# OedonLestrange42/GNURadio-WiFI-ImageTransfer

Measured on NVIDIA B200. Metric: rx_msamples_per_s, higher is better.
Workload: dtype f32+u8

## Files before the change

### gnuradio-wifi-imagetransfer_b200/csrc/rx_kernels.cuh

```cuda
#pragma once
#include <cuda_pipeline.h>
#include "viterbi.cuh"

__device__ __forceinline__ cf fe_at(const cf *x, int64_t j, int hist) { return j < -(int64_t)hist ? cf{0.f, 0.f} : x[j]; }

__device__ __forceinline__ int find_link(const LinkDesc *links, int n_links, int64_t chunk)
{
    int lo = 0, hi = n_links - 1;
    while (lo < hi) {
        int mid = (lo + hi + 1) >> 1;
        if (links[mid].chunk_base <= chunk) lo = mid; else hi = mid - 1;
    }
    return lo;
}

#ifndef DET_BLOCK
#define DET_BLOCK 32
#endif
#define DET_SPLIT (DET_THREADS / DET_BLOCK)
#define DET_ROWS (DET_BLOCK + 2)
#define DET_STRIDE 66
#define DET_SMEM_BYTES (DET_ROWS * DET_STRIDE * (int)sizeof(cf) + 32)

__device__ __forceinline__ uint32_t det_smem_u32(const void *p) { return (uint32_t)__cvta_generic_to_shared(p); }
// ... 775 lines not shown
                        if (k == 32 || k < 6 || k > 58) continue;
                        sum = cadd(sum, s_hu[wib][k]);
                        ++cnt;
                    }
                    cf avg = {sum.re / (float)cnt, sum.im / (float)cnt};
                    if (u) HB = cadd(cscale(HB, 0.5f), cscale(avg, 0.5f));
                    else HA = cadd(cscale(HA, 0.5f), cscale(avg, 0.5f));
                }
                __syncwarp();
            }
            if (PHASE == 0) {
                if (carA >= 0) st->sig_bits[carA] = (uint8_t)bitsA;
                if (carB >= 0) st->sig_bits[carB] = (uint8_t)bitsB;
            } else {
                int64_t row = F.row_off + (n - 3);
                if (carA >= 0) rows[row * 48 + carA] = (uint8_t)bitsA;
                if (carB >= 0) rows[row * 48 + carB] = (uint8_t)bitsB;
                if (prm.want_carrier) {
                    if (carA >= 0) carrier[row * 48 + carA] = symA;
                    if (carB >= 0) carrier[row * 48 + carB] = symB;
                }
                if (wps) {
                    if (carA >= 0)
                        *reinterpret_cast<uint2 *>(&s_bits[wib][carA * 8]) =
                            make_uint2((((uint32_t)bitsA & 15u) * 0x00204081u) & 0x01010101u, (((uint32_t)bitsA >> 4) * 0x81u) & 0x0101u);
                    if (carB >= 0)
                        *reinterpret_cast<uint2 *>(&s_bits[wib][carB * 8]) =
                            make_uint2((((uint32_t)bitsB & 15u) * 0x00204081u) & 0x01010101u, (((uint32_t)bitsB >> 4) * 0x81u) & 0x0101u);
                    __syncwarp();
                    if (lane < wps) {
                        uint32_t word = era_word;
#pragma unroll
                        for (int j = 0; j < 4; ++j) {
                            const uint4 e = reinterpret_cast<const uint4 *>(s_lut[wib])[j * 27 + lane];
                            word += ((uint32_t)s_bits[wib][e.x] << (8 * j)) + ((uint32_t)s_bits[wib][e.y] << (8 * j + 2)) +
                                    ((uint32_t)s_bits[wib][e.z] << (8 * j + 4)) + ((uint32_t)s_bits[wib][e.w] << (8 * j + 6));
                        }
                        vw[(n - 3) * wps + lane] = word;
                    }
                    __syncwarp();
                }
                if (SOFT && soft_on) {
                    const int hb = nb > 1 ? nb >> 1 : 1;
#pragma unroll
                    for (int u = 0; u < 2; ++u)
#pragma unroll
                        for (int t = 0; t < 3; ++t) {
                            if (t < hb && (u == 0 || nb > 1)) {
                                const int k = u * hb + t;
                                if (carA >= 0) { s_soft[wib][(carA << 3) | k] = (int8_t)sqA.q[u][t]; soft_rows[row * SOFT_ROW + carA * nb + k] = (int8_t)sqA.q[u][t]; }
                                if (carB >= 0) { s_soft[wib][(carB << 3) | k] = (int8_t)sqB.q[u][t]; soft_rows[row * SOFT_ROW + carB * nb + k] = (int8_t)sqB.q[u][t]; }
                            }
                        }
                    __syncwarp();
                    for (int w = lane; w < swps; w += 32) {
                        uint32_t word = 0;
#pragma unroll
                        for (int k = 0; k < 4; ++k) word |= (uint32_t)(uint8_t)s_soft[wib][s_slut[wib][4 * w + k]] << (8 * k);
                        vsw[(n - 3) * swps + w] = word;
                    }
                    __syncwarp();
                }
                ++n_rows;
            }
        }
    }
    if (phase == 0) {
        st->H[iA] = HA; st->H[iB] = HB;
        if (SOFT) { st->w0[iA] = w0A; st->w0[iB] = w0B; }
        if (lane == 0) {
#pragma unroll
            for (int q = 0; q < 4; ++q) st->prev_pil[q] = pp[q];
            st->d_er = d_er; st->eps0 = eps0; st->snr = snr; st->havg = havg;
        }
    } else if (lane == 0) {
        frames[f].n_rows = n_rows;
    }
}

__global__ void __launch_bounds__(VIT_BLOCK) k_signal(wifi_b200_frame *frames, int f0, int n_frames, const EqState *states)
{
    __shared__ uint32_t ring[5 * 16 * VIT_BLOCK];
    __shared__ uint4 s_bm[8 * 4 * 16];
    const int tid = threadIdx.x;
    for (int i = tid; i < 512; i += VIT_BLOCK) s_bm[i] = VitCoreH::table_entry(i >> 6, (i >> 4) & 3, (uint32_t)(i & 15));
    __syncthreads();
    int f = f0 + blockIdx.x * VIT_BLOCK + tid;
    if (f >= n_frames) return;
    if (frames[f].n_syms < 3) return;
    const EqState *st = states + f;
    uint64_t lo = 0, hi = 0;
    for (int tstep = 0; tstep < 24; ++tstep) {
        int i0 = 2 * tstep, i1 = i0 + 1;
        uint32_t s0 = st->sig_bits[(i0 % 16) * 3 + i0 / 16] & 1u, s1 = st->sig_bits[(i1 % 16) * 3 + i1 / 16] & 1u;
        uint64_t nib = s0 | (s1 << 2);
        if (tstep < 16) lo |= nib << (4 * tstep); else hi |= nib << (4 * (tstep - 16));
    }
    VitCoreH v;
    v.init();
    const uint32_t first = (uint32_t)lo;
    v.step4<0>(s_bm, 0xau, 0xau, first & 0xfu, (first >> 4) & 0xfu);
    v.step4<4>(s_bm, (first >> 8) & 0xfu, (first >> 12) & 0xfu, (first >> 16) & 0xfu, (first >> 20) & 0xfu);
    v.trace_begin(ring, 1, 5, tid, true, 0xfcu);
    uint32_t dec = 0;
#pragma unroll 1
    for (int chunk = 1; chunk < 8; ++chunk) {
        const uint32_t bits = (uint32_t)(lo >> 24);
        lo = (lo >> 32) | (hi << 32);
        hi >>= 32;
        v.step4<0>(s_bm, bits & 0xfu, (bits >> 4) & 0xfu, (bits >> 8) & 0xfu, (bits >> 12) & 0xfu);
        v.step4<4>(s_bm, (bits >> 16) & 0xfu, (bits >> 20) & 0xfu, (bits >> 24) & 0xfu, bits >> 28);
        VitTrace tr = v.trace_begin(ring, (chunk + 1) % 5, 5, tid, (chunk & 3) == 0);
        if (chunk >= 5) {
            VitCoreH::trace_hops<4>(tr, ring, 5, tid);
            dec |= vit_ring_byte(ring, tr.sl, tr.bs, tid) << (8 * (chunk - 5));
        }
    }
    int r = 0, len = 0;
    bool parity = false;
    for (int i = 0; i < 17; ++i) {
        bool bit = (dec >> i) & 1u;
        parity ^= bit;
        if (i < 4 && bit) r |= 1 << i;
        if (bit && i > 4) len |= 1 << (i - 5);
    }
    if (parity != (bool)((dec >> 17) & 1u)) return;
    int enc;
    switch (r) {
    case 11: enc = 0; break;
    case 15: enc = 1; break;
    case 10: enc = 2; break;
    case 14: enc = 3; break;
    case 9: enc = 4; break;
    case 13: enc = 5; break;
    case 8: enc = 6; break;
    case 12: enc = 7; break;
    default: return;
    }
    int ndbps = c_tab.mcs[enc].n_dbps;
    frames[f].sig_ok = 1;
    frames[f].encoding = enc;
    frames[f].length = len;
    frames[f].frame_symbols = (16 + 8 * len + 6 + ndbps - 1) / ndbps;
    frames[f].snr = st->snr;
}

struct PlanState { int cur, copied, need, pending; JobDesc J; };

__device__ void plan_sequential(PlanState &S, int f0, int f1, wifi_b200_frame *frames, JobDesc *jobs, int *pack_list, int *n_pack, int *err, int soft)
{
    for (int fi = f0; fi < f1; ++fi) {
        wifi_b200_frame F = frames[fi];
        if (!F.sig_ok) continue;
        if (F.n_rows == 0) {
            if (S.pending < 0) S.pending = fi;
            continue;
        }
        int tagf = S.pending >= 0 ? S.pending : fi;
        S.pending = -1;
        int t_sym = frames[tagf].frame_symbols, t_len = frames[tagf].length;
        if (t_sym <= WIFI_MAX_SYM && t_len <= WIFI_MAX_PSDU) {
            frames[tagf].accepted = 1;
            S.cur = tagf;
            S.copied = 0;
            S.need = t_sym;
            S.J.frame = tagf; S.J.enc = frames[tagf].encoding; S.J.len = t_len; S.J.n_sym = t_sym; S.J.n_seg = 0; S.J.need_pack = 0;
        }
        if (S.cur < 0 || S.copied >= S.need) continue;
        int take = F.n_rows < S.need - S.copied ? F.n_rows : S.need - S.copied;
        if (S.J.n_seg < 4) {
            S.J.seg_row[S.J.n_seg] = (int32_t)F.row_off;
            S.J.seg_cnt[S.J.n_seg] = take;
        }
        S.J.n_seg++;
        S.copied += take;
        if (S.copied == S.need) {
            S.J.last_frame = fi;
            S.J.pad0 = 0;
            for (int s = S.J.n_seg; s < 4; ++s) { S.J.seg_row[s] = 0; S.J.seg_cnt[s] = 0; }
            bool own = (S.J.n_seg == 1 && fi == S.cur);
            S.J.need_pack = (!own || (!soft && (c_tab.mcs[S.J.enc].n_dbps & 7) != 0)) ? 1 : 0;
            jobs[S.cur] = S.J;
            if (S.J.need_pack) pack_list[atomicAdd(n_pack, 1)] = S.cur;
            frames[S.cur].decoded = 1;
            frames[S.cur].psdu_off = (int64_t)S.cur * PSDU_STRIDE;
        }
    }
}

__global__ void __launch_bounds__(128) k_plan_fast(wifi_b200_frame *frames, int f0, int n_frames, JobDesc *jobs, int *pack_list, int *n_pack,
                                                    int *link_dirty, int soft)
{
    int fi = f0 + blockIdx.x * blockDim.x + threadIdx.x;
    if (fi >= n_frames) return;
    const wifi_b200_frame *F = frames + fi;
    const int sig = F->sig_ok, nrows = F->n_rows, fsym = F->frame_symbols, len = F->length, enc = F->encoding;
    jobs[fi].n_sym = 0;
    if (!sig) return;
// ... 40 lines not shown
        bool quiet = !valid || !sig;
        bool all_simple = __all_sync(0xffffffffu, regular || quiet);
        if (all_simple && S.pending < 0) {
            if (regular) {
                JobDesc J;
                J.frame = fi; J.enc = enc; J.len = len; J.n_sym = fsym; J.n_seg = 1;
                J.seg_row[0] = (int32_t)row_off; J.seg_cnt[0] = fsym;
                for (int s = 1; s < 4; ++s) { J.seg_row[s] = 0; J.seg_cnt[s] = 0; }
                J.need_pack = (!soft && (c_tab.mcs[enc].n_dbps & 7) != 0) ? 1 : 0;
                J.last_frame = fi; J.pad0 = 0;
                jobs[fi] = J;
                if (J.need_pack) pack_list[atomicAdd(n_pack, 1)] = fi;
                frames[fi].accepted = 1;
                frames[fi].decoded = 1;
                frames[fi].psdu_off = (int64_t)fi * PSDU_STRIDE;
            }
            unsigned reg = __ballot_sync(0xffffffffu, regular);
            if (reg) {
                int lastl = 31 - __clz((int)reg);
                S.cur = f0 + lastl;
                S.need = __shfl_sync(0xffffffffu, fsym, lastl);
                S.copied = S.need;
                S.J.n_seg = 0;
            }
        } else {
            __syncwarp();
            if (lane == 0) plan_sequential(S, f0, f0 + 32 < fend ? f0 + 32 : fend, frames, jobs, pack_list, n_pack, err, soft);
            S.cur = __shfl_sync(0xffffffffu, S.cur, 0);
            S.copied = __shfl_sync(0xffffffffu, S.copied, 0);
            S.need = __shfl_sync(0xffffffffu, S.need, 0);
            S.pending = __shfl_sync(0xffffffffu, S.pending, 0);
        }
    }
    if (lane == 0) link_open[l] = S.pending >= 0 ? S.pending : ((S.cur >= 0 && S.copied < S.need) ? S.cur : -1);
}

__global__ void __launch_bounds__(256) k_pack(const JobDesc *__restrict__ jobs, const int *__restrict__ pack_list, const int *__restrict__ n_pack,
                                               const uint8_t *__restrict__ rows, const uint16_t *__restrict__ depunct_lut, uint32_t *__restrict__ vit_in,
                                               const wifi_b200_frame *__restrict__ frames)
{
    const int np = *n_pack;
    for (int e = blockIdx.y; e < np; e += gridDim.y) {
        const JobDesc J = jobs[pack_list[e]];
        if (J.n_sym == 0 || !J.need_pack) continue;
        const int ndbps = c_tab.mcs[J.enc].n_dbps;
        const int per = 2 * ndbps;
        const int n_data = J.n_sym * ndbps;
        const int n_words = (n_data + 7) >> 3;
        const uint16_t *lut = depunct_lut + J.enc * 432;
        uint32_t *vw = vit_in + (int64_t)J.frame * VIT_MAXW;
        for (int w = blockIdx.x * blockDim.x + threadIdx.x; w < n_words; w += gridDim.x * blockDim.x) {
            int tstep = 8 * w;
            int q = 2 * tstep;
            int s = q / per, qi = q - s * per;
            const uint8_t *rp = rows + job_row(J, frames, s) * 48;
            uint32_t word = 0;
#pragma unroll
            for (int k = 0; k < 16; ++k) {
                uint32_t sym = 0;
                if (tstep + (k >> 1) < n_data) {
                    uint16_t en = lut[qi];
                    sym = (en == 0xffffu) ? 2u : ((rp[en >> 3] >> (en & 7)) & 1u);
                }
                word |= sym << (2 * k);
                if (++qi == per) {
                    qi = 0;
                    ++s;
                    if (s < J.n_sym) rp = rows + job_row(J, frames, s) * 48;
                }
            }
            vw[w] = word;
        }
    }
}

__global__ void __launch_bounds__(VIT_BLOCK) k_viterbi(const JobDesc *__restrict__ jobs, int f0, int n_frames, const uint32_t *__restrict__ vit_in,
                                                        uint32_t *__restrict__ psdu, wifi_b200_frame *frames)
{
    extern __shared__ uint32_t vsm[];
    uint32_t *ring = vsm;
    uint32_t *s_crc = vsm + VIT_NTB_MAX * 16 * VIT_BLOCK;
    uint16_t *s_scr = (uint16_t *)(s_crc + 256);
    uint4 *s_bm = (uint4 *)(s_crc + 256 + 64);
    const int tid = threadIdx.x;
    for (int i = tid; i < 256; i += VIT_BLOCK) s_crc[i] = c_tab.crc_tab[i];
    for (int i = tid; i < 128; i += VIT_BLOCK) s_scr[i] = c_tab.scr_tab[i];
    for (int i = tid; i < 512; i += VIT_BLOCK) s_bm[i] = VitCoreH::table_entry(i >> 6, (i >> 4) & 3, (uint32_t)(i & 15));
    __syncthreads();
    const int job = f0 + blockIdx.x * VIT_BLOCK + tid;
    if (job >= n_frames) return;
    const JobDesc J = jobs[job];
    if (J.n_sym == 0) return;
    const int punct = c_tab.mcs[J.enc].punct;
    const int ntb = punct == 0 ? 5 : (punct == 1 ? 9 : 10);
    const int nw = (J.n_sym * c_tab.mcs[J.enc].n_dbps + 7) >> 3;
    const uint32_t *in = vit_in + (int64_t)job * VIT_MAXW;
    uint32_t *out = psdu + (int64_t)job * (PSDU_STRIDE / 4);
    const int L = J.len;
    const int last_chunk = L + 1 + ntb;
    VitCoreH v;
    v.init();
    uint32_t prev = in[0];
    v.step4<0>(s_bm, 0xau, 0xau, prev & 0xfu, (prev >> 4) & 0xfu);
    v.step4<4>(s_bm, (prev >> 8) & 0xfu, (prev >> 12) & 0xfu, (prev >> 16) & 0xfu, (prev >> 20) & 0xfu);
    int slot = 1 % ntb;
    v.trace_begin(ring, slot, ntb, tid, true, 0xfcu);
    PsduSink sink;
    sink.init(out, L, s_crc, s_scr);
    uint32_t next = 1 < nw ? in[1] : 0u;
    VitTrace tr;
    tr.bs = 0; tr.sl = slot; tr.left = 0;
    bool pending = false;
#pragma unroll 1
    for (int chunk = 1; chunk <= last_chunk; ++chunk) {
        uint32_t bits = __funnelshift_r(prev, next, 24);
        prev = next;
        next = (chunk + 1 < nw) ? in[chunk + 1] : 0u;
        VitCoreH::trace_hops<3>(tr, ring, ntb, tid);
        v.step4<0>(s_bm, bits & 0xfu, (bits >> 4) & 0xfu, (bits >> 8) & 0xfu, (bits >> 12) & 0xfu);
        VitCoreH::trace_hops<3>(tr, ring, ntb, tid);
        v.step4<4>(s_bm, (bits >> 16) & 0xfu, (bits >> 20) & 0xfu, (bits >> 24) & 0xfu, bits >> 28);
        VitCoreH::trace_hops<3>(tr, ring, ntb, tid);
        if (pending && chunk - 1 >= ntb) sink.push(VitCoreH::trace_finish(tr, ring, tid), chunk - 1 - ntb);
        slot = (slot + 1 == ntb) ? 0 : slot + 1;
        tr = v.trace_begin(ring, slot, ntb, tid, (chunk & 3) == 0);
        pending = true;
    }
    if (pending && last_chunk >= ntb) {
        VitCoreH::trace_hops<9>(tr, ring, ntb, tid);
        sink.push(VitCoreH::trace_finish(tr, ring, tid), last_chunk - ntb);
    }
    frames[J.frame].crc_ok = sink.crc_ok();
}

__global__ void __launch_bounds__(VQ_BLOCK) k_viterbi_quad(const JobDesc *__restrict__ jobs, int f0, int n_frames, const uint32_t *__restrict__ vit_in,
                                                          uint32_t *__restrict__ psdu, wifi_b200_frame *frames)
{
    __shared__ uint32_t s_ring[VQ_FRAMES * VQ_RSTRIDE];
    __shared__ uint32_t s_crc[256];
    __shared__ uint16_t s_scr[128];
    __shared__ uint2 s_bm[16];
    const int tid = threadIdx.x;
    for (int i = tid; i < 256; i += VQ_BLOCK) s_crc[i] = c_tab.crc_tab[i];
    for (int i = tid; i < 128; i += VQ_BLOCK) s_scr[i] = c_tab.scr_tab[i];
    if (tid < 16) { uint32_t T, E; VitQuad::branch((uint32_t)tid, T, E); s_bm[tid] = make_uint2(T, E); }
    __syncthreads();
    const int job = f0 + blockIdx.x * VQ_FRAMES + (tid >> 2);
    JobDesc J;
    J.n_sym = 0;
    if (job < n_frames) J = jobs[job];
    const bool active = job < n_frames && J.n_sym != 0;
    if (!__any_sync(0xffffffffu, active)) return;
    const int enc = active ? J.enc : 0;
    const int punct = c_tab.mcs[enc].punct;
    const int ntb = punct == 0 ? 5 : (punct == 1 ? 9 : 10);
    const int nw = active ? (J.n_sym * c_tab.mcs[enc].n_dbps + 7) >> 3 : 0;
    const uint32_t *in = vit_in + (int64_t)(active ? job : f0) * VIT_MAXW;
    const int L = active ? J.len : 0;
    const int last_chunk = active ? L + 1 + ntb : 0;
    const int trips = __reduce_max_sync(0xffffffffu, last_chunk);
    uint32_t *ring = s_ring + (tid >> 2) * VQ_RSTRIDE;
    VitQuad v;
    v.init(tid & 31);
    uint32_t prev = 0 < nw ? in[0] : 0u;
    v.step4<0>(s_bm, 0xau, 0xau, prev & 0xfu, (prev >> 4) & 0xfu);
    v.step4<4>(s_bm, (prev >> 8) & 0xfu, (prev >> 12) & 0xfu, (prev >> 16) & 0xfu, (prev >> 20) & 0xfu);
#pragma unroll
    for (int i = 0; i < 4; ++i) v.p[i] &= 0x3f3f3f3fu;
    int slot = 1 % ntb;
    v.trace_begin(ring, slot, ntb, true);
    PsduSink sink;
    sink.init(psdu + (int64_t)(active ? job : f0) * (PSDU_STRIDE / 4), L, s_crc, s_scr);
    sink.writer = active && (tid & 3) == 0;
    uint32_t next = 1 < nw ? in[1] : 0u;
    VitTrace tr;
    tr.bs = 0; tr.sl = slot; tr.left = 0;
#pragma unroll 1
    for (int chunk = 1; chunk <= trips; ++chunk) {
        const uint32_t bits = __funnelshift_r(prev, next, 24);
        prev = next;
        next = (chunk + 1 < nw) ? in[chunk + 1] : 0u;
        VitQuad::trace_hops<3>(tr, ring, ntb);
        v.step4<0>(s_bm, bits & 0xfu, (bits >> 4) & 0xfu, (bits >> 8) & 0xfu, (bits >> 12) & 0xfu);
        VitQuad::trace_hops<3>(tr, ring, ntb);
        v.step4<4>(s_bm, (bits >> 16) & 0xfu, (bits >> 20) & 0xfu, (bits >> 24) & 0xfu, bits >> 28);
        VitQuad::trace_hops<3>(tr, ring, ntb);
        if (chunk - 1 >= ntb && chunk - 1 <= last_chunk) sink.push(VitQuad::ring_byte(ring, tr.sl, tr.bs), chunk - 1 - ntb);
        slot = (slot + 1 == ntb) ? 0 : slot + 1;
        tr = v.trace_begin(ring, slot, ntb, (chunk & 3) == 0);
    }
    VitQuad::trace_hops<9>(tr, ring, ntb);
    if (trips == last_chunk && last_chunk >= ntb) sink.push(VitQuad::ring_byte(ring, tr.sl, tr.bs), last_chunk - ntb);
    if (sink.writer) frames[J.frame].crc_ok = sink.crc_ok();
}

#define VW_WARPS 4
#define VW_RING 48
__global__ void __launch_bounds__(32 * VW_WARPS) k_viterbi_warp(const JobDesc *__restrict__ jobs, int f0, int n_frames, const uint32_t *__restrict__ vit_in,
                                                               uint32_t *__restrict__ psdu, wifi_b200_frame *frames)
{
    __shared__ uint8_t s_ring[VW_WARPS][VW_RING][64];
    __shared__ uint32_t s_keys[VW_WARPS][32 * 33];
    __shared__ uint32_t s_crc[256];
    __shared__ uint16_t s_scr[128];
    for (int i = threadIdx.x; i < 256; i += blockDim.x) s_crc[i] = c_tab.crc_tab[i];
    for (int i = threadIdx.x; i < 128; i += blockDim.x) s_scr[i] = c_tab.scr_tab[i];
    __syncthreads();
    const int wib = threadIdx.x >> 5, lane = threadIdx.x & 31;
    const int job = f0 + blockIdx.x * VW_WARPS + wib;
    if (job >= n_frames) return;
    const JobDesc J = jobs[job];
    if (J.n_sym == 0) return;
    const int punct = c_tab.mcs[J.enc].punct;
// ... 156 lines not shown
```

### gnuradio-wifi-imagetransfer_b200/csrc/viterbi.cuh

```cuda
#pragma once
#include "wifi_common.cuh"

#define VIT_BLOCK 64
#define VIT_NTB_MAX 10

__device__ __forceinline__ uint32_t prmt(uint32_t a, uint32_t b, uint32_t sel)
{
    uint32_t d;
    asm("prmt.b32 %0, %1, %2, %3;" : "=r"(d) : "r"(a), "r"(b), "r"(sel));
    return d;
}

__host__ __device__ constexpr uint32_t vit_par(uint32_t v) { return (v ^ (v >> 1) ^ (v >> 2) ^ (v >> 3) ^ (v >> 4) ^ (v >> 5) ^ (v >> 6)) & 1u; }
__host__ __device__ constexpr uint32_t vit_sel2(int k0, int k1)
{
    const int k[2] = {k0, k1};
    uint32_t s = 0;
    for (int b = 0; b < 2; ++b) {
        uint32_t idx = 2 * vit_par((2 * k[b]) & 0x6d) + vit_par((2 * k[b]) & 0x4f);
        s |= ((2 * idx) | ((2 * idx + 1) << 4)) << (8 * b);
    }
    return s;
}

struct VitTrace { int bs, sl, left; };
__device__ __forceinline__ uint32_t vit_ring_byte(const uint32_t *ring, int sl, int bs, int tid)
{
    const uint8_t *rb = reinterpret_cast<const uint8_t *>(ring) + tid * 4;
    return rb[sl * (16 * VIT_BLOCK * 4) + (bs >> 2) * (VIT_BLOCK * 4) + (bs & 3)];
}

struct VitCoreH {
    uint32_t X[32];

    __device__ __forceinline__ void init()
    {
#pragma unroll
        for (int i = 0; i < 32; ++i) X[i] = 0;
    }
    static __device__ __forceinline__ uint4 branch(uint32_t nib)
    {
        const uint32_t s0 = nib & 3u, s1 = (nib >> 2) & 3u;
        const uint32_t e0 = s0 != 2u, e1 = s1 != 2u;
        uint32_t t[4];
#pragma unroll
        for (uint32_t p = 0; p < 4; ++p) t[p] = ((e0 & (s0 ^ (p >> 1))) + (e1 & (s1 ^ (p & 1u)))) << 8;
        return make_uint4(t[0] | (t[1] << 16), t[2] | (t[3] << 16), ((e0 + e1) << 8) * 0x00010001u, 0u);
    }
    static __device__ __forceinline__ uint32_t fadd(uint32_t a, uint32_t b)
    {
        uint32_t d;
        asm("mad.lo.u32 %0, %1, 1, %2;" : "=r"(d) : "r"(a), "r"(b));
        return d;
    }
    static __device__ __forceinline__ uint4 table_entry(int s, int c, uint32_t nib)
    {
        const int st = s & 3;
        const int c1 = st == 0 ? (c ^ 1) : (st == 3 ? c : 3 - c);
        const uint32_t sel = (uint32_t)((2 * c) | ((2 * c + 1) << 4)) | ((uint32_t)((2 * c1) | ((2 * c1 + 1) << 4)) << 8);
        const uint4 b = branch(nib);
        const uint32_t svm = prmt(b.x, b.y, sel), sv = b.z - svm, bit = 0x00010001u << s;
        return make_uint4(svm, sv, svm + bit, sv + bit);
    }
    static __device__ __forceinline__ void bflyt(const uint4 e, uint32_t lo, uint32_t hi, uint32_t &v0, uint32_t &v1)
    {
        v0 = __viaddmax_u16x2(lo, e.y, fadd(hi, e.z));
        v1 = __viaddmax_u16x2(lo, e.x, fadd(hi, e.w));
    }
    static __host__ __device__ constexpr int selc(uint32_t sel) { return (int)((sel & 0xfu) >> 1); }
    template <int S0>
    __device__ __forceinline__ void step4(const uint4 *bt, uint32_t n0, uint32_t n1, uint32_t n2, uint32_t n3)
    {
        uint32_t S[32], Q[32];
        uint4 e[4];
#pragma unroll
        for (int c = 0; c < 4; ++c) e[c] = bt[((S0 + 0) * 4 + c) * 16 + n0];
#pragma unroll
        for (int j = 0; j < 16; ++j) bflyt(e[selc(vit_sel2(2 * j, 2 * j + 1))], X[j], X[j + 16], S[j], S[16 + j]);
#pragma unroll
        for (int c = 0; c < 4; ++c) e[c] = bt[((S0 + 1) * 4 + c) * 16 + n1];
#pragma unroll
        for (int j = 0; j < 8; ++j) {
            bflyt(e[selc(vit_sel2(4 * j, 4 * j + 2))], S[j], S[j + 8], Q[4 * j], Q[4 * j + 1]);
            bflyt(e[selc(vit_sel2(4 * j + 1, 4 * j + 3))], S[16 + j], S[24 + j], Q[4 * j + 2], Q[4 * j + 3]);
        }
#pragma unroll
        for (int c = 0; c < 4; ++c) e[c] = bt[((S0 + 2) * 4 + c) * 16 + n2];
#pragma unroll
        for (int j = 0; j < 4; ++j)
#pragma unroll
            for (int o = 0; o < 4; ++o)
                bflyt(e[selc(vit_sel2(8 * j + o, 8 * j + 4 + o))], Q[4 * j + o], Q[4 * (j + 4) + o], S[8 * j + 2 * o], S[8 * j + 2 * o + 1]);
#pragma unroll
        for (int c = 0; c < 4; ++c) e[c] = bt[((S0 + 3) * 4 + c) * 16 + n3];
#pragma unroll
        for (int j = 0; j < 2; ++j)
#pragma unroll
            for (int o = 0; o < 8; ++o)
                bflyt(e[selc(vit_sel2(16 * j + o, 16 * j + 8 + o))], S[8 * j + o], S[8 * (j + 2) + o], Q[16 * j + 2 * o], Q[16 * j + 2 * o + 1]);
#pragma unroll
        for (int j = 0; j < 2; ++j)
#pragma unroll
            for (int e2 = 0; e2 < 16; e2 += 2) {
                X[(32 * j + e2) >> 1] = prmt(Q[16 * j + e2], Q[16 * j + e2 + 1], 0x5410u);
                X[(32 * j + 16 + e2) >> 1] = prmt(Q[16 * j + e2], Q[16 * j + e2 + 1], 0x7632u);
            }
    }
    __device__ __forceinline__ VitTrace trace_begin(uint32_t *ring, int slot, int ntb, int tid, bool renorm, uint32_t keep = 0xffu)
    {
        const uint32_t keepw = 0xff00ff00u | keep | (keep << 16);
#pragma unroll
        for (int w = 0; w < 16; ++w) ring[(slot * 16 + w) * VIT_BLOCK + tid] = prmt(X[2 * w] & keepw, X[2 * w + 1] & keepw, 0x6420u);
        uint32_t key[32];
#pragma unroll
        for (int j = 0; j < 32; ++j) {
            X[j] &= 0xff00ff00u;
            key[j] = fadd(X[j], (uint32_t)(63 - 2 * j) | ((uint32_t)(62 - 2 * j) << 16));
        }
#pragma unroll
        for (int n = 16; n >= 1; n >>= 1)
#pragma unroll
            for (int i = 0; i < n; ++i) key[i] = __vmaxu2(key[i], key[i + n]);
        const uint32_t kbest = max(key[0] & 0xffffu, key[0] >> 16);
        VitTrace t;
        t.bs = 63 - (int)(kbest & 0xffu);
        t.sl = slot;
        t.left = ntb - 1;
        if (renorm) {
            const uint32_t mx = kbest >> 8;
            const uint32_t nminw = 0u - (mx > 12u ? ((mx - 12u) << 8) * 0x00010001u : 0u);
#pragma unroll
            for (int i = 0; i < 32; ++i) X[i] = fadd(X[i], nminw);
        }
        return t;
    }
    template <int N>
    static __device__ __forceinline__ void trace_hops(VitTrace &t, const uint32_t *ring, int ntb, int tid)
    {
#pragma unroll
        for (int i = 0; i < N; ++i) {
            const bool go = t.left > 0;
            const int nb = (int)(__brev(vit_ring_byte(ring, t.sl, t.bs, tid)) >> 26);
            const int ns = (t.sl == 0) ? ntb - 1 : t.sl - 1;
            t.bs = go ? nb : t.bs;
            t.sl = go ? ns : t.sl;
            t.left -= go ? 1 : 0;
        }
    }
    static __device__ __forceinline__ uint32_t trace_finish(const VitTrace &t, const uint32_t *ring, int tid)
    {
        return __brev(vit_ring_byte(ring, t.sl, t.bs, tid)) >> 24;
    }
};

#define VQ_BLOCK 64
#define VQ_FRAMES (VQ_BLOCK / 4)
#define VQ_RSTRIDE (VIT_NTB_MAX * 16 + 4)

struct VitQuad {
    uint32_t m[4], p[4];
    uint32_t selA0, selA1, selB0, selB1, selC0, selC1, selD0, selD1;
    uint32_t keyc[4];
    int g;
    bool hiC, hiD;

    static __device__ __forceinline__ void branch(uint32_t nib, uint32_t &T, uint32_t &E)
    {
        const uint32_t s0 = nib & 3u, s1 = (nib >> 2) & 3u;
        const uint32_t t0 = (s0 == 2u) ? 0u : (s0 ? 0x00000101u : 0x01010000u);
        const uint32_t t1 = (s1 == 2u) ? 0u : (s1 ? 0x00010001u : 0x01000100u);
        T = t0 + t1;
        E = ((s0 != 2u) ? 0x01010101u : 0u) + ((s1 != 2u) ? 0x01010101u : 0u);
    }
    static __device__ __forceinline__ uint32_t sel4(int k0, int k1, int k2, int k3)
    {
        const int k[4] = {k0, k1, k2, k3};
        uint32_t s = 0;
#pragma unroll
        for (int b = 0; b < 4; ++b) {
            const uint32_t A = __popc((2u * k[b]) & 0x6du) & 1u, B = __popc((2u * k[b]) & 0x4fu) & 1u;
            s |= (2 * A + B) << (4 * b);
        }
        return s;
    }

    __device__ __forceinline__ void init(int lane_in_warp)
    {
        g = lane_in_warp & 3;
#pragma unroll
        for (int i = 0; i < 4; ++i) { m[i] = 0; p[i] = 0; keyc[i] = 0x3c3d3e3fu - 0x04040404u * (uint32_t)(g + 4 * i); }
        selA0 = sel4(4 * g, 4 * g + 1, 4 * g + 2, 4 * g + 3);
        selA1 = sel4(4 * (g + 4), 4 * (g + 4) + 1, 4 * (g + 4) + 2, 4 * (g + 4) + 3);
        selB0 = sel4(8 * g, 8 * g + 2, 8 * g + 4, 8 * g + 6);
        selB1 = sel4(8 * g + 1, 8 * g + 3, 8 * g + 5, 8 * g + 7);
        hiC = (g >> 1) != 0;
        { const int j = g & 1, o = hiC ? 2 : 0;
          selC0 = sel4(16 * j + o, 16 * j + 4 + o, 16 * j + 8 + o, 16 * j + 12 + o);
          selC1 = sel4(16 * j + o + 1, 16 * j + 5 + o, 16 * j + 9 + o, 16 * j + 13 + o); }
        hiD = (g & 1) != 0;
        { const int o = (g >> 1) * 4 + (g & 1) * 2;
          selD0 = sel4(o, 8 + o, 16 + o, 24 + o);
          selD1 = sel4(o + 1, 9 + o, 17 + o, 25 + o); }
    }

    template <uint32_t BIT>
    static __device__ __forceinline__ void bfly(uint32_t T, uint32_t E, uint32_t sel, uint32_t lo, uint32_t hi, uint32_t plo, uint32_t phi,
                                                uint32_t &v0, uint32_t &v1, uint32_t &q0, uint32_t &q1)
    {
        const uint32_t svm = prmt(T, 0u, sel), sv = E - svm;
        const uint32_t m0 = lo + sv, m1 = hi + svm, m2 = lo + svm, m3 = hi + sv;
        const uint32_t k0 = prmt(m0 + 0x7f7f7f7fu - m1, 0u, 0xba98u);
        const uint32_t k1 = prmt(m2 + 0x7f7f7f7fu - m3, 0u, 0xba98u);
        v0 = (m0 & k0) | (m1 & ~k0);
        v1 = (m2 & k1) | (m3 & ~k1);
        const uint32_t pb = phi + BIT;
        q0 = (plo & k0) | (pb & ~k0);
        q1 = (plo & k1) | (pb & ~k1);
    }

    __device__ __forceinline__ void exchange(const uint32_t (&x)[4], bool high, int lane_xor, uint32_t &lo_a, uint32_t &hi_a, uint32_t &lo_b, uint32_t &hi_b) const
    {
        const uint32_t ra = __shfl_xor_sync(0xffffffffu, high ? x[0] : x[2], lane_xor);
        const uint32_t rb = __shfl_xor_sync(0xffffffffu, high ? x[1] : x[3], lane_xor);
        lo_a = high ? ra : x[0]; hi_a = high ? x[2] : ra;
        lo_b = high ? rb : x[1]; hi_b = high ? x[3] : rb;
    }

    template <int S0>
    __device__ __forceinline__ void step4(const uint2 *bm, uint32_t n0, uint32_t n1, uint32_t n2, uint32_t n3)
    {
        constexpr uint32_t B0 = 0x01010101u << (7 - S0), B1 = B0 >> 1, B2 = B0 >> 2, B3 = B0 >> 3;
        uint32_t T, E;
        uint32_t s[4], sp[4], q[4], qp[4];
        { const uint2 te = bm[n0]; T = te.x; E = te.y; }
        bfly<B0>(T, E, selA0, m[0], m[2], p[0], p[2], s[0], s[2], sp[0], sp[2]);
// ... 240 lines not shown
```

### gnuradio-wifi-imagetransfer_b200/csrc/wifi_b200.cu

```cuda
#include <sched.h>

#include <cfloat>
#include <cmath>
#include <cstdio>
#include <cstdlib>
#include <cstring>
#include <mutex>
#include <string>
#include <deque>
#include <vector>

#include "rx_kernels.cuh"
#include "tx_kernels.cuh"


namespace {

const McsDesc H_MCS[8] = {
    {1, 48, 24, 0x0D, 0}, {1, 48, 36, 0x0F, 2}, {2, 96, 48, 0x05, 0}, {2, 96, 72, 0x07, 2},
    {4, 192, 96, 0x09, 0}, {4, 192, 144, 0x0B, 2}, {6, 288, 192, 0x01, 1}, {6, 288, 216, 0x03, 2},
};
const int H_LTS53[53] = {1, 1, -1, -1, 1, 1, -1, 1, -1, 1, 1, 1, 1, 1, 1, -1, -1, 1, 1, -1, 1, -1, 1, 1, 1, 1, 0,
                         1, -1, -1, 1, 1, -1, 1, -1, 1, -1, -1, -1, -1, -1, 1, 1, -1, -1, 1, -1, 1, -1, 1, 1, 1, 1};

// ... 43 lines not shown
        t.tw[k].im = (float)(-std::sin(2.0 * M_PI * k / 64.0));
    }
    t.tw[0] = {1.f, 0.f};
    t.tw[16] = {0.f, -1.f};
    t.win = (float)(1.0 / std::sqrt(52.0));
    const float sv = (float)std::sqrt(13.0 / 6.0);
    const int sts_k[12] = {-24, -20, -16, -12, -8, -4, 4, 8, 12, 16, 20, 24};
    const int sts_s[12] = {1, -1, 1, -1, -1, 1, -1, -1, 1, 1, 1, 1};
    for (int i = 0; i < 12; ++i) t.sts[sts_k[i] + 32] = {sts_s[i] * sv, sts_s[i] * sv};
    for (int i = 0; i < 64; ++i) {
        int k = i - 32, m = ((k % 4) + 4) % 4;
        float v = t.lts[i];
        t.lts_rot[i] = (m == 0) ? cf{v, 0.f} : (m == 1) ? cf{0.f, -v} : (m == 2) ? cf{-v, 0.f} : cf{0.f, v};
    }
    for (int e = 0; e < 8; ++e) {
        t.mcs[e] = H_MCS[e];
        int n_cbps = H_MCS[e].n_cbps, s = std::max(H_MCS[e].n_bpsc / 2, 1);
        int first[288], second[288];
        for (int j = 0; j < n_cbps; ++j) first[j] = s * (j / s) + ((j + (int)std::floor(16.0 * j / n_cbps)) % s);
        for (int i = 0; i < n_cbps; ++i) second[i] = 16 * i - (n_cbps - 1) * (int)std::floor(16.0 * i / n_cbps);
        for (int k = 0; k < n_cbps; ++k) {
            t.P[e][k] = (uint16_t)second[first[k]];
            t.Pinv[e][second[first[k]]] = (uint16_t)k;
        }
        int nb = H_MCS[e].n_bpsc;
        for (int v = 0; v < (1 << nb); ++v) {
            if (nb == 1) { t.cons[e][v] = {v ? 1.f : -1.f, 0.f}; continue; }
            int h = nb / 2;
            float level = (h == 1) ? sqrtf(0.5f) : (h == 2) ? sqrtf(0.1f) : sqrtf(1.0f / 42.0f);
            auto axis = [&](int bits) -> float {
                int b0 = bits & 1, b1 = (bits >> 1) & 1, b2 = (bits >> 2) & 1, mag;
                if (h == 1) mag = 1;
                else if (h == 2) mag = b1 ? 1 : 3;
                else mag = b1 ? (b2 ? 3 : 1) : (b2 ? 5 : 7);
                return (float)(b0 ? mag : -mag) * level;
            };
            t.cons[e][v] = {axis(v & ((1 << h) - 1)), axis(v >> h)};
        }
    }
    h_crc_init();
    memcpy(t.crc_tab, h_crc_tab, sizeof h_crc_tab);
    for (int s0 = 0; s0 < 128; ++s0) {
        int st = s0, fbits = 0;
        for (int i = 0; i < 8; ++i) {
            int fb = ((st >> 6) & 1) ^ ((st >> 3) & 1);
            fbits |= fb << i;
            st = ((st << 1) & 0x7e) | fb;
        }
        t.scr_tab[s0] = (uint16_t)(fbits | (st << 8));
    }
    int c = 0;
    for (int i = 0; i < 64; ++i) {
        if (i < 6 || i > 58 || i == 32 || i == 11 || i == 25 || i == 39 || i == 53) t.carrier_of[i] = -1;
        else t.carrier_of[i] = (int8_t)c++;
    }
    depunct.assign(8 * 432, 0xffff);
    for (int e = 0; e < 8; ++e) {
        const McsDesc &m = H_MCS[e];
        int per = 2 * m.n_dbps, cb = 0;
        for (int q = 0; q < per; ++q) {
            bool keep = true;
            if (m.punct == 1) keep = (q % 4) != 3;
            else if (m.punct == 2) keep = !((q % 6) == 3 || (q % 6) == 4);
            if (!keep) continue;
            int k = t.Pinv[e][cb];
            depunct[e * 432 + q] = (uint16_t)(((k / m.n_bpsc) << 3) | (k % m.n_bpsc));
            ++cb;
        }
    }
}

enum { ST_H2D = 0, ST_DETECT, ST_SELECT, ST_SYNC_LONG, ST_DEMOD_HEAD, ST_SIGNAL, ST_DEMOD_DATA, ST_PLAN, ST_PACK, ST_VITERBI, ST_D2H, ST_COUNT };
const char *STAGE_NAMES[ST_COUNT] = {"h2d", "detect", "select", "sync_long", "demod_head", "signal", "demod_data", "plan", "pack", "viterbi", "d2h"};

#define MAX_LINKS 16384
#ifndef VW_SWITCH
#define VW_SWITCH 1280
#endif
#ifndef VQ_SWITCH
#define VQ_SWITCH 10240
#endif
#define VQ_SPLIT_MAX 4736
#define DET_SMEM DET_SMEM_BYTES
#define VIT_SMEM_BYTES ((VIT_NTB_MAX * 16 * VIT_BLOCK + 256) * 4 + 256 + 8192)

}


#define A_SLOTS 3
struct wifi_b200 {
    wifi_b200_cfg cfg;
    int device = 0;
    cudaStream_t stream = nullptr;
    cudaStream_t copy_stream = nullptr, d2h_stream = nullptr;
    cudaStream_t aux_stream = nullptr;
    cudaEvent_t ev_fork = nullptr, ev_join = nullptr;
    int sm_count = 148;
    std::vector<cudaEvent_t> ev_h2d, ev_done;
    std::mutex mu;
    std::string err;
    cf *d_iq = nullptr;
    int16_t *d_sc16 = nullptr;
    uint32_t *d_flags = nullptr;
    uint32_t *d_summary = nullptr;
    int *d_trig_tmp = nullptr;
    int *d_spec_trig = nullptr;
    int4 *d_spec_cnt = nullptr;
    int *d_spec_trig2 = nullptr;
    int4 *d_spec_cnt2 = nullptr;
    int *d_pack_list = nullptr;
    int *d_link_dirty = nullptr;
    int64_t tile_cap = 0;
    LinkDesc *d_links = nullptr;
    wifi_b200_frame *d_frames = nullptr;
    EqState *d_states = nullptr;
    uint8_t *d_rows = nullptr;
    cf *d_carrier = nullptr;
    JobDesc *d_jobs = nullptr;
    uint32_t *d_vit_in = nullptr;
    int8_t *d_soft = nullptr;
    uint32_t *d_vit_soft_in = nullptr;
    uint32_t *d_psdu = nullptr;
    uint16_t *d_depunct = nullptr;
    int *d_counters = nullptr;
    int *h_counters = nullptr;
    int64_t row_cap = 0;
    uint8_t *d_txblob = nullptr;
    TxFrameDesc *d_txdesc = nullptr;
    uint8_t *d_txsym = nullptr;
    cf *d_txiq = nullptr;
    size_t txblob_cap = 0, txiq_cap = 0, txsym_cap = 0;
    int64_t tx_sym_bytes = 0;
    int tx_seed = 1;
    wifi_b200_chan_seg *d_segs = nullptr;
    wifi_b200_fading *d_fades = nullptr;
    size_t segs_cap = 0, fades_cap = 0;
    const cf *cur_iq = nullptr;
    std::vector<LinkDesc> h_links;
    int64_t n_frames = 0, n_jobs = 0, n_rows = 0, n_samples = 0, n_triggers = 0;
    bool host_mirror = false;
    bool psdu_mirror = false;
    wifi_b200_frame *h_frames = nullptr;
    uint8_t *h_psdu = nullptr;
    float *h_iq = nullptr;
    cudaEvent_t ev[ST_COUNT + 1];
    bool ev_used[ST_COUNT + 1];
    float stage_ms[ST_COUNT];
    wifi_b200_stats stats;
    struct StreamLink {
        int64_t fill = 0;
        int64_t abs0 = 0;
        int hist = 0;
        int64_t prev_trigger = -1;
        float fo_carry = 0.f;
    };
    std::vector<StreamLink> s_links;
    cf *d_stream = nullptr;
    int64_t s_cap = 0;
    struct MoveSeg { int64_t src, dst, n; };
    MoveSeg *d_moves = nullptr;
    int64_t group_samples = 0;
    int64_t s_batch = 0;
    int64_t s_unprocessed = 0;
    struct StreamBlock { uint8_t *buf = nullptr; std::vector<wifi_b200_frame> meta; size_t next = 0; };
    std::vector<wifi_b200_frame> s_meta;
    std::vector<uint8_t> s_bytes;
    std::deque<StreamBlock> s_blocks;
// ... 1435 lines not shown
```

Baseline: 49690.

## Precompute Viterbi traceback hop addresses via shared lookup tables

Replaces the traceback state (slot, bit-state, remaining count) with a single shared-memory byte address. Each hop is now two dependent shared loads, a ring byte followed by a precomputed offset table entry. Per-ntb slot row tables replace the modular slot arithmetic and the 'left' predication, with an identity slot padding the shorter traceback depths. The survivor snapshot is taken from Q before the butterfly permute, with the permute fused into trace_begin. This shortens the latency-bound traceback chain but adds shared-memory tables, keeps Q live in registers, and raises register pressure.

```diff
diff --git a/gnuradio-wifi-imagetransfer_b200/csrc/rx_kernels.cuh b/gnuradio-wifi-imagetransfer_b200/csrc/rx_kernels.cuh
--- a/gnuradio-wifi-imagetransfer_b200/csrc/rx_kernels.cuh
+++ b/gnuradio-wifi-imagetransfer_b200/csrc/rx_kernels.cuh
@@ -881,8 +881,10 @@
 {
     __shared__ uint32_t ring[5 * 16 * VIT_BLOCK];
     __shared__ uint4 s_bm[8 * 4 * 16];
+    __shared__ uint32_t s_hop[VIT_HOP_ENTRIES];
     const int tid = threadIdx.x;
     for (int i = tid; i < 512; i += VIT_BLOCK) s_bm[i] = VitCoreH::table_entry(i >> 6, (i >> 4) & 3, (uint32_t)(i & 15));
+    for (int i = tid; i < VIT_HOP_ENTRIES; i += VIT_BLOCK) s_hop[i] = vit_h_hop_entry(i);
     __syncthreads();
     int f = f0 + blockIdx.x * VIT_BLOCK + tid;
     if (f >= n_frames) return;
@@ -900,7 +902,9 @@
     const uint32_t first = (uint32_t)lo;
     v.step4<0>(s_bm, 0xau, 0xau, first & 0xfu, (first >> 4) & 0xfu);
     v.step4<4>(s_bm, (first >> 8) & 0xfu, (first >> 12) & 0xfu, (first >> 16) & 0xfu, (first >> 20) & 0xfu);
-    v.trace_begin(ring, 1, 5, tid, true, 0xfcu);
+    uint8_t *rbt = reinterpret_cast<uint8_t *>(ring) + 4 * tid;
+    const uint32_t rbt_sh = (uint32_t)__cvta_generic_to_shared(rbt), hop_sh = (uint32_t)__cvta_generic_to_shared(s_hop);
+    v.trace_begin(rbt + VIT_SLOT_BYTES, rbt_sh + VIT_SLOT_BYTES, s_hop, true, 0xfcu);
     uint32_t dec = 0;
 #pragma unroll 1
     for (int chunk = 1; chunk < 8; ++chunk) {
@@ -909,10 +913,15 @@
         hi >>= 32;
         v.step4<0>(s_bm, bits & 0xfu, (bits >> 4) & 0xfu, (bits >> 8) & 0xfu, (bits >> 12) & 0xfu);
         v.step4<4>(s_bm, (bits >> 16) & 0xfu, (bits >> 20) & 0xfu, (bits >> 24) & 0xfu, bits >> 28);
-        VitTrace tr = v.trace_begin(ring, (chunk + 1) % 5, 5, tid, (chunk & 3) == 0);
+        int sl = (chunk + 1) % 5;
+        uint32_t c = v.trace_begin(rbt + sl * VIT_SLOT_BYTES, rbt_sh + sl * VIT_SLOT_BYTES, s_hop, (chunk & 3) == 0);
         if (chunk >= 5) {
-            VitCoreH::trace_hops<4>(tr, ring, 5, tid);
-            dec |= vit_ring_byte(ring, tr.sl, tr.bs, tid) << (8 * (chunk - 5));
+            asm volatile("" ::: "memory");
+            for (int i = 0; i < 4; ++i) {
+                sl = sl == 0 ? 4 : sl - 1;
+                c = VitCoreH::hop(c, hop_sh, rbt_sh + sl * VIT_SLOT_BYTES);
+            }
+            dec |= VitCoreH::ring_byte(c) << (8 * (chunk - 5));
         }
     }
     int r = 0, len = 0;
@@ -1119,10 +1128,15 @@
     uint32_t *s_crc = vsm + VIT_NTB_MAX * 16 * VIT_BLOCK;
     uint16_t *s_scr = (uint16_t *)(s_crc + 256);
     uint4 *s_bm = (uint4 *)(s_crc + 256 + 64);
+    uint4 *s_rows = s_bm + 512;
+    uint32_t *s_hop = (uint32_t *)(s_rows + 3 * VIT_ROWS);
     const int tid = threadIdx.x;
     for (int i = tid; i < 256; i += VIT_BLOCK) s_crc[i] = c_tab.crc_tab[i];
     for (int i = tid; i < 128; i += VIT_BLOCK) s_scr[i] = c_tab.scr_tab[i];
     for (int i = tid; i < 512; i += VIT_BLOCK) s_bm[i] = VitCoreH::table_entry(i >> 6, (i >> 4) & 3, (uint32_t)(i & 15));
+    for (int i = tid; i < 12 * VIT_ROWS; i += VIT_BLOCK) ((uint32_t *)s_rows)[i] = vit_h_row_entry(i / 12, i % 12);
+    for (int i = tid; i < VIT_HOP_ENTRIES; i += VIT_BLOCK) s_hop[i] = vit_h_hop_entry(i);
+    for (int w = 0; w < 16; ++w) ring[(VIT_ID_SLOT * 16 + w) * VIT_BLOCK + tid] = vit_h_identity_word(w);
     __syncthreads();
     const int job = f0 + blockIdx.x * VIT_BLOCK + tid;
     if (job >= n_frames) return;
@@ -1140,32 +1154,42 @@
     uint32_t prev = in[0];
     v.step4<0>(s_bm, 0xau, 0xau, prev & 0xfu, (prev >> 4) & 0xfu);
     v.step4<4>(s_bm, (prev >> 8) & 0xfu, (prev >> 12) & 0xfu, (prev >> 16) & 0xfu, (prev >> 20) & 0xfu);
-    int slot = 1 % ntb;
-    v.trace_begin(ring, slot, ntb, tid, true, 0xfcu);
+    uint8_t *rbt = reinterpret_cast<uint8_t *>(ring) + 4 * tid;
+    const uint32_t rbt_sh = (uint32_t)__cvta_generic_to_shared(rbt), hop_sh = (uint32_t)__cvta_generic_to_shared(s_hop);
+    int row = 3 * (vit_h_row0(ntb) + 1);
+    uint4 r0 = s_rows[row];
+    uint32_t c = v.trace_begin(rbt + r0.x, rbt_sh + r0.y, s_hop, true, 0xfcu);
     PsduSink sink;
     sink.init(out, L, s_crc, s_scr);
     uint32_t next = 1 < nw ? in[1] : 0u;
-    VitTrace tr;
-    tr.bs = 0; tr.sl = slot; tr.left = 0;
-    bool pending = false;
 #pragma unroll 1
     for (int chunk = 1; chunk <= last_chunk; ++chunk) {
         uint32_t bits = __funnelshift_r(prev, next, 24);
         prev = next;
         next = (chunk + 1 < nw) ? in[chunk + 1] : 0u;
-        VitCoreH::trace_hops<3>(tr, ring, ntb, tid);
+        const uint4 r1 = s_rows[row + 1], r2 = s_rows[row + 2];
+        c = VitCoreH::hop(c, hop_sh, rbt_sh + r0.z);
+        c = VitCoreH::hop(c, hop_sh, rbt_sh + r0.w);
+        c = VitCoreH::hop(c, hop_sh, rbt_sh + r1.x);
         v.step4<0>(s_bm, bits & 0xfu, (bits >> 4) & 0xfu, (bits >> 8) & 0xfu, (bits >> 12) & 0xfu);
-        VitCoreH::trace_hops<3>(tr, ring, ntb, tid);
+        c = VitCoreH::hop(c, hop_sh, rbt_sh + r1.y);
+        c = VitCoreH::hop(c, hop_sh, rbt_sh + r1.z);
+        c = VitCoreH::hop(c, hop_sh, rbt_sh + r1.w);
         v.step4<4>(s_bm, (bits >> 16) & 0xfu, (bits >> 20) & 0xfu, (bits >> 24) & 0xfu, bits >> 28);
-        VitCoreH::trace_hops<3>(tr, ring, ntb, tid);
-        if (pending && chunk - 1 >= ntb) sink.push(VitCoreH::trace_finish(tr, ring, tid), chunk - 1 - ntb);
-        slot = (slot + 1 == ntb) ? 0 : slot + 1;
-        tr = v.trace_begin(ring, slot, ntb, tid, (chunk & 3) == 0);
-        pending = true;
-    }
-    if (pending && last_chunk >= ntb) {
-        VitCoreH::trace_hops<9>(tr, ring, ntb, tid);
-        sink.push(VitCoreH::trace_finish(tr, ring, tid), last_chunk - ntb);
+        c = VitCoreH::hop(c, hop_sh, rbt_sh + r2.x);
+        c = VitCoreH::hop(c, hop_sh, rbt_sh + r2.y);
+        c = VitCoreH::hop(c, hop_sh, rbt_sh + r2.z);
+        if (chunk - 1 >= ntb) sink.push(VitCoreH::trace_finish(c), chunk - 1 - ntb);
+        row = (int)r2.w;
+        r0 = s_rows[row];
+        c = v.trace_begin(rbt + r0.x, rbt_sh + r0.y, s_hop, (chunk & 3) == 0);
+    }
+    if (last_chunk >= ntb) {
+        const uint4 r1 = s_rows[row + 1], r2 = s_rows[row + 2];
+        const uint32_t base[9] = {r0.z, r0.w, r1.x, r1.y, r1.z, r1.w, r2.x, r2.y, r2.z};
+#pragma unroll
+        for (int i = 0; i < 9; ++i) c = VitCoreH::hop(c, hop_sh, rbt_sh + base[i]);
+        sink.push(VitCoreH::trace_finish(c), last_chunk - ntb);
     }
     frames[J.frame].crc_ok = sink.crc_ok();
 }
diff --git a/gnuradio-wifi-imagetransfer_b200/csrc/viterbi.cuh b/gnuradio-wifi-imagetransfer_b200/csrc/viterbi.cuh
--- a/gnuradio-wifi-imagetransfer_b200/csrc/viterbi.cuh
+++ b/gnuradio-wifi-imagetransfer_b200/csrc/viterbi.cuh
@@ -30,8 +30,47 @@
     return rb[sl * (16 * VIT_BLOCK * 4) + (bs >> 2) * (VIT_BLOCK * 4) + (bs & 3)];
 }
 
+__host__ __device__ constexpr uint32_t vit_h_off(uint32_t x)
+{
+    return (8 * (x >> 5) + ((x & 15) >> 1)) * (VIT_BLOCK * 4) + ((x >> 4) & 1) + 2 * (x & 1);
+}
+#define VIT_SLOT_BYTES (16 * VIT_BLOCK * 4)
+#define VIT_HOP_ENTRIES (256 + 64)
+__device__ __forceinline__ uint32_t vit_h_hop_entry(int i)
+{
+    return vit_h_off(i < 256 ? __brev((uint32_t)i) >> 26 : 63u - (uint32_t)(i - 256));
+}
+__device__ __forceinline__ uint32_t vit_h_identity_word(int w)
+{
+    const uint32_t j = (uint32_t)w >> 3, m = 2u * ((uint32_t)w & 7u);
+    const uint32_t x[4] = {32 * j + m, 32 * j + 16 + m, 32 * j + m + 1, 32 * j + m + 17};
+    uint32_t v = 0;
+#pragma unroll
+    for (int k = 0; k < 4; ++k) v |= (__brev(x[k]) >> 26) << (8 * k);
+    return v;
+}
+
+#define VIT_ROWS 24
+#define VIT_ID_SLOT 9
+static_assert(VIT_NTB_MAX == 10 && VIT_ID_SLOT == VIT_NTB_MAX - 1, "traceback rows assume ntb in {5, 9, 10}, ten ring slots");
+__host__ __device__ constexpr int vit_h_row0(int ntb) { return ntb == 5 ? 0 : (ntb == 9 ? 5 : 14); }
+__device__ __forceinline__ uint32_t vit_h_row_entry(int r, int e)
+{
+    const int ntb = r < 5 ? 5 : (r < 14 ? 9 : 10);
+    const int s = r - vit_h_row0(ntb);
+    int slot;
+    if (e == 0) slot = s;
+    else if (e == 1) slot = ntb == 10 ? s : VIT_ID_SLOT;
+    else if (e <= 10) {
+        const int still = 10 - ntb, i = e - 2;
+        slot = i < still - 1 ? VIT_ID_SLOT : (s - (i - still + 1) + ntb) % ntb;
+    } else return (uint32_t)(3 * (vit_h_row0(ntb) + (s + 1) % ntb));
+    return (uint32_t)(slot * VIT_SLOT_BYTES);
+}
+
 struct VitCoreH {
     uint32_t X[32];
+    uint32_t Q[32];
 
     __device__ __forceinline__ void init()
     {
@@ -71,7 +110,7 @@
     template <int S0>
     __device__ __forceinline__ void step4(const uint4 *bt, uint32_t n0, uint32_t n1, uint32_t n2, uint32_t n3)
     {
-        uint32_t S[32], Q[32];
+        uint32_t S[32];
         uint4 e[4];
 #pragma unroll
         for (int c = 0; c < 4; ++c) e[c] = bt[((S0 + 0) * 4 + c) * 16 + n0];
@@ -98,59 +137,61 @@
 #pragma unroll
             for (int o = 0; o < 8; ++o)
                 bflyt(e[selc(vit_sel2(16 * j + o, 16 * j + 8 + o))], S[8 * j + o], S[8 * (j + 2) + o], Q[16 * j + 2 * o], Q[16 * j + 2 * o + 1]);
+        if (S0 == 0) {
+#pragma unroll
+            for (int j = 0; j < 2; ++j)
+#pragma unroll
+                for (int e2 = 0; e2 < 16; e2 += 2) {
+                    X[(32 * j + e2) >> 1] = prmt(Q[16 * j + e2], Q[16 * j + e2 + 1], 0x5410u);
+                    X[(32 * j + 16 + e2) >> 1] = prmt(Q[16 * j + e2], Q[16 * j + e2 + 1], 0x7632u);
+                }
+        }
+    }
+    __device__ __forceinline__ uint32_t trace_begin(uint8_t *snap, uint32_t c0_base, const uint32_t *hop_tab, bool renorm,
+                                                    uint32_t keep = 0xffu)
+    {
+        const uint32_t keepw = 0xff00ff00u | keep | (keep << 16);
+#pragma unroll
+        for (int w = 0; w < 16; ++w)
+            *reinterpret_cast<uint32_t *>(snap + w * (VIT_BLOCK * 4)) = prmt(Q[2 * w] & keepw, Q[2 * w + 1] & keepw, 0x6420u);
 #pragma unroll
         for (int j = 0; j < 2; ++j)
 #pragma unroll
             for (int e2 = 0; e2 < 16; e2 += 2) {
-                X[(32 * j + e2) >> 1] = prmt(Q[16 * j + e2], Q[16 * j + e2 + 1], 0x5410u);
-                X[(32 * j + 16 + e2) >> 1] = prmt(Q[16 * j + e2], Q[16 * j + e2 + 1], 0x7632u);
+                X[(32 * j + e2) >> 1] = prmt(Q[16 * j + e2], Q[16 * j + e2 + 1], 0x5d19u);
+                X[(32 * j + 16 + e2) >> 1] = prmt(Q[16 * j + e2], Q[16 * j + e2 + 1], 0x7f3bu);
             }
-    }
-    __device__ __forceinline__ VitTrace trace_begin(uint32_t *ring, int slot, int ntb, int tid, bool renorm, uint32_t keep = 0xffu)
-    {
-        const uint32_t keepw = 0xff00ff00u | keep | (keep << 16);
-#pragma unroll
-        for (int w = 0; w < 16; ++w) ring[(slot * 16 + w) * VIT_BLOCK + tid] = prmt(X[2 * w] & keepw, X[2 * w + 1] & keepw, 0x6420u);
         uint32_t key[32];
 #pragma unroll
-        for (int j = 0; j < 32; ++j) {
-            X[j] &= 0xff00ff00u;
-            key[j] = fadd(X[j], (uint32_t)(63 - 2 * j) | ((uint32_t)(62 - 2 * j) << 16));
-        }
+        for (int j = 0; j < 32; ++j) key[j] = fadd(X[j], (uint32_t)(63 - 2 * j) | ((uint32_t)(62 - 2 * j) << 16));
 #pragma unroll
         for (int n = 16; n >= 1; n >>= 1)
 #pragma unroll
             for (int i = 0; i < n; ++i) key[i] = __vmaxu2(key[i], key[i + n]);
         const uint32_t kbest = max(key[0] & 0xffffu, key[0] >> 16);
-        VitTrace t;
-        t.bs = 63 - (int)(kbest & 0xffu);
-        t.sl = slot;
-        t.left = ntb - 1;
+        const uint32_t c = c0_base + hop_tab[256 + (kbest & 0xffu)];
         if (renorm) {
             const uint32_t mx = kbest >> 8;
             const uint32_t nminw = 0u - (mx > 12u ? ((mx - 12u) << 8) * 0x00010001u : 0u);
 #pragma unroll
             for (int i = 0; i < 32; ++i) X[i] = fadd(X[i], nminw);
         }
-        return t;
-    }
-    template <int N>
-    static __device__ __forceinline__ void trace_hops(VitTrace &t, const uint32_t *ring, int ntb, int tid)
-    {
-#pragma unroll
-        for (int i = 0; i < N; ++i) {
-            const bool go = t.left > 0;
-            const int nb = (int)(__brev(vit_ring_byte(ring, t.sl, t.bs, tid)) >> 26);
-            const int ns = (t.sl == 0) ? ntb - 1 : t.sl - 1;
-            t.bs = go ? nb : t.bs;
-            t.sl = go ? ns : t.sl;
-            t.left -= go ? 1 : 0;
-        }
-    }
-    static __device__ __forceinline__ uint32_t trace_finish(const VitTrace &t, const uint32_t *ring, int tid)
-    {
-        return __brev(vit_ring_byte(ring, t.sl, t.bs, tid)) >> 24;
-    }
+        return c;
+    }
+    static __device__ __forceinline__ uint32_t hop(uint32_t c, uint32_t hop_tab, uint32_t base)
+    {
+        uint32_t b, t;
+        asm volatile("ld.shared.u8 %0, [%1];" : "=r"(b) : "r"(c));
+        asm("ld.shared.u32 %0, [%1];" : "=r"(t) : "r"(hop_tab + 4u * b));
+        return base + t;
+    }
+    static __device__ __forceinline__ uint32_t ring_byte(uint32_t c)
+    {
+        uint32_t b;
+        asm volatile("ld.shared.u8 %0, [%1];" : "=r"(b) : "r"(c) : "memory");
+        return b;
+    }
+    static __device__ __forceinline__ uint32_t trace_finish(uint32_t c) { return __brev(ring_byte(c)) >> 24; }
 };
 
 #define VQ_BLOCK 64
diff --git a/gnuradio-wifi-imagetransfer_b200/csrc/wifi_b200.cu b/gnuradio-wifi-imagetransfer_b200/csrc/wifi_b200.cu
--- a/gnuradio-wifi-imagetransfer_b200/csrc/wifi_b200.cu
+++ b/gnuradio-wifi-imagetransfer_b200/csrc/wifi_b200.cu
@@ -149,7 +149,7 @@
 #endif
 #define VQ_SPLIT_MAX 4736
 #define DET_SMEM DET_SMEM_BYTES
-#define VIT_SMEM_BYTES ((VIT_NTB_MAX * 16 * VIT_BLOCK + 256) * 4 + 256 + 8192)
+#define VIT_SMEM_BYTES ((VIT_NTB_MAX * 16 * VIT_BLOCK + 256) * 4 + 256 + 8192 + VIT_ROWS * 48 + VIT_HOP_ENTRIES * 4)
 
 }
 
```

After: 52770, median of 6. +6.2%, better.
